# zacharie12/Hypernet-image-captioning

Hardware: AMD Instinct MI355X
Metric: training images/sec at 1/2/4/8 MI355X, Flickr30k GRU+hypernet bs=128 (higher is better)
Workload: dtype f32; 1 GPU; Flickr30k-shaped GRU+additive-attention decoder + hypernet (3 style domains), full training step (fwd, CE, bwd, clip 5.0, Adam); per_gpu_batch=128, global_batch=128, T=20, P=49, D=2048, F=200, E=200, H=200, V=9684, hypernet_params=144906720, parallelism=dp1, launch=eager, next_theta_in_adam_pass=True, next_precompute_beside_adam=True, spinup_steps=0, deterministic_gradients=True

## Files before the change

hypernet-image-captioning_amd/csrc/misc.hip:

```cpp
#include "common.h"
#include "gemm_internal.h"
#include <math.h>

namespace {
constexpr int RMAX = 8;


__global__ __launch_bounds__(256) void ce_count_kernel(int rows, const int64_t* __restrict__ tgt, int64_t ignore, float* nvalid) {
    __shared__ int cnt[4];
    int c = 0;
    for (int i = threadIdx.x; i < rows; i += 256) c += (tgt[i] != ignore);
    float cf = wave_sum((float)c);
    if ((threadIdx.x & 63) == 0) cnt[threadIdx.x >> 6] = (int)cf;
    __syncthreads();
    if (threadIdx.x == 0) nvalid[0] = (float)(cnt[0] + cnt[1] + cnt[2] + cnt[3]);
}

__global__ __launch_bounds__(256) void ce_row_kernel(int V, int ld, const float* logits, const int64_t* __restrict__ tgt,
                                                     int64_t ignore, const float* __restrict__ nvalid, const int* __restrict__ nvi,
                                                     float* dlogits, float* __restrict__ row_loss, int vec) {
    __shared__ float red[4];
    __shared__ float bc[2];
    const int row = blockIdx.x, tid = threadIdx.x;
    const float* x = logits + (size_t)row * ld;
// ... 300 lines not shown
        } else {
            for (size_t i = base + tid; i < n && i < base + SUMSQ_CHUNK; i += 256) s += x[i] * x[i];
        }
        mine = (double)s;
    } else {
        int q = bid - nb_s;
        const int chunk = q % NORM_CHUNKS; q /= NORM_CHUNKS;
        const int pair = q % (R * R); q /= (R * R);
        const int which = q & 1, job = q >> 1;
        const GramJob& J = jobs.j[job];
        const int r = pair / R, sidx = pair % R;
        const float* u = which ? J.afac + (size_t)r * J.lda : J.gfac + (size_t)r * J.ldg;
        const float* v = which ? J.afac + (size_t)sidx * J.lda : J.gfac + (size_t)sidx * J.ldg;
        const int len = which ? J.k : J.rows;
        const int per = (len + NORM_CHUNKS - 1) / NORM_CHUNKS;
        const int i0 = chunk * per, i1 = min(len, i0 + per);
        int i = i0 + tid;
        for (; i + 7 * 256 < i1; i += 8 * 256) {
            float uu[8], vv[8];
#pragma unroll
            for (int e = 0; e < 8; ++e) { uu[e] = u[i + 256 * e]; vv[e] = v[i + 256 * e]; }
#pragma unroll
            for (int e = 0; e < 8; ++e) mine += (double)uu[e] * (double)vv[e];
        }
        for (; i < i1; i += 256) mine += (double)u[i] * (double)v[i];
    }
    mine = wave_sum_d(mine);
    if ((tid & 63) == 0) red[tid >> 6] = mine;
    __syncthreads();
    if (tid == 0) part[bid] = red[0] + red[1] + red[2] + red[3];
}
__device__ __forceinline__ float norm_finish(int nb_s, int R, int njobs, const double* __restrict__ part, double max_norm, double scale,
                                             double* red , float* norm_out) {
    const int tid = threadIdx.x;
    const double* gram = part + nb_s;
    double tot = 0.0;
    for (int i = tid; i < nb_s; i += 256) tot += part[i];
    const int npair = njobs * R * R;
    for (int i = tid; i < npair; i += 256) {
        const int job = i / (R * R), pair = i % (R * R);
        const double* gg = gram + (((size_t)job * 2 + 0) * R * R + pair) * NORM_CHUNKS;
        const double* aa = gram + (((size_t)job * 2 + 1) * R * R + pair) * NORM_CHUNKS;
        double sg = 0.0, sa = 0.0;
        for (int c = 0; c < NORM_CHUNKS; ++c) { sg += gg[c]; sa += aa[c]; }
        tot += sg * sa;
    }
    tot = wave_sum_d(tot);
    if ((tid & 63) == 0) red[tid >> 6] = tot;
    __syncthreads();
    const double t = red[0] + red[1] + red[2] + red[3];
    const double norm = scale * sqrt(t);
    double c = max_norm / (norm + 1e-6);
    if (c > 1.0) c = 1.0;
    *norm_out = (float)norm;
    return (float)(scale * c);
}
__global__ __launch_bounds__(256) void grad_norm_finish_kernel(int nb_s, int R, int njobs, const double* __restrict__ part,
                                                               double max_norm, double scale, float* __restrict__ coef_out) {
    __shared__ double red[5];
    float norm;
    const float c = norm_finish(nb_s, R, njobs, part, max_norm, scale, red, &norm);
    if (threadIdx.x == 0) { coef_out[0] = c; coef_out[1] = norm; }
}

struct AdamK { float lr_bc1, b1, b2, eps, sqrt_bc2; const float* dev; int zg = 0; };
__device__ __forceinline__ void adam_moments(float g, float& m, float& v, const AdamK& k) {
    m = m + (g - m) * (1.0f - k.b1);
    v = v * k.b2 + (1.0f - k.b2) * g * g;
}
__device__ __forceinline__ float adam_elem(float p, float g, float& m, float& v, const AdamK& k) {
    adam_moments(g, m, v, k);
    const float denom = sqrtf(v) / k.sqrt_bc2 + k.eps;
    return p - k.lr_bc1 * (m / denom);
}
__device__ __forceinline__ void adam_moments_rank1(float a, float r, float& m, float& v, const AdamK& k) {
#pragma clang fp contract(off)
    const float g = a * r;
    const float d = __builtin_fmaf(a, r, -m);
    m = __builtin_fmaf(1.0f - k.b1, d, m);
    const float t = (1.0f - k.b2) * g;
    const float vb = v * k.b2, tg = t * g;
    v = vb + tg;
}
__device__ __forceinline__ float adam_elem_rank1(float p, float a, float r, float& m, float& v, const AdamK& k) {
#pragma clang fp contract(off)
    adam_moments_rank1(a, r, m, v, k);
    const float denom = sqrtf(v) / k.sqrt_bc2 + k.eps;
    return __builtin_fmaf(-k.lr_bc1, m / denom, p);
}
__global__ __launch_bounds__(256) void adam_dense_kernel(size_t n, float* __restrict__ p, float* __restrict__ m, float* __restrict__ v,
                                                         const float* __restrict__ g, const float* __restrict__ coef, AdamK k, int vec) {
    const float c = coef[0];
    if (k.dev) { k.lr_bc1 = k.dev[0]; k.sqrt_bc2 = k.dev[1]; }
    const size_t stride = (size_t)gridDim.x * 256;
    if (vec) {
        f32x4* p4 = reinterpret_cast<f32x4*>(p); f32x4* m4 = reinterpret_cast<f32x4*>(m); f32x4* v4 = reinterpret_cast<f32x4*>(v);
        const f32x4* g4 = reinterpret_cast<const f32x4*>(g);
        const size_t n4 = n >> 2;
        for (size_t i = (size_t)blockIdx.x * 256 + threadIdx.x; i < n4; i += stride) {
            f32x4 pp = p4[i], mm = m4[i], vv = v4[i], gg = g4[i];
#pragma unroll
            for (int e = 0; e < 4; ++e) { float me = mm[e], ve = vv[e]; pp[e] = adam_elem(pp[e], gg[e] * c, me, ve, k); mm[e] = me; vv[e] = ve; }
            p4[i] = pp; m4[i] = mm; v4[i] = vv;
        }
        for (size_t i = (n4 << 2) + (size_t)blockIdx.x * 256 + threadIdx.x; i < n; i += stride) {
            float me = m[i], ve = v[i]; p[i] = adam_elem(p[i], g[i] * c, me, ve, k); m[i] = me; v[i] = ve;
        }
    } else {
        for (size_t i = (size_t)blockIdx.x * 256 + threadIdx.x; i < n; i += stride) {
            float me = m[i], ve = v[i]; p[i] = adam_elem(p[i], g[i] * c, me, ve, k); m[i] = me; v[i] = ve;
        }
    }
}

struct NormFin { const double* part; int nb_s, R, njobs; double max_norm, scale; float* coef_out;
                 int ce_rows; const float* ce_rowloss; const float* ce_nvalid; const int* ce_nvi; float* loss_out; };
__global__ __launch_bounds__(256) void adam_dense_clip_kernel(size_t n, float* __restrict__ p, float* __restrict__ m, float* __restrict__ v,
                                                              const float* __restrict__ g, NormFin nf, AdamK k, int vec) {
    __shared__ double red[5];
    float norm;
    const float c = norm_finish(nf.nb_s, nf.R, nf.njobs, nf.part, nf.max_norm, nf.scale, red, &norm);
    if (blockIdx.x == 0) {
        if (threadIdx.x == 0) { nf.coef_out[0] = c; nf.coef_out[1] = norm; }
        if (nf.ce_rows > 0) {
            __syncthreads();
            double s = 0.0;
            for (int i = threadIdx.x; i < nf.ce_rows; i += 256) s += (double)nf.ce_rowloss[i];
            s = wave_sum_d(s);
            if ((threadIdx.x & 63) == 0) red[threadIdx.x >> 6] = s;
            __syncthreads();
            if (threadIdx.x == 0) {
                const float nn = nf.ce_nvi ? (float)nf.ce_nvi[0] : nf.ce_nvalid[0];
                nf.loss_out[0] = (float)((red[0] + red[1] + red[2] + red[3]) / (double)nn); nf.loss_out[1] = nn;
            }
        }
    }
    if (k.dev) { k.lr_bc1 = k.dev[0]; k.sqrt_bc2 = k.dev[1]; }
    const size_t stride = (size_t)gridDim.x * 256;
    if (vec) {
        f32x4* p4 = reinterpret_cast<f32x4*>(p); f32x4* m4 = reinterpret_cast<f32x4*>(m); f32x4* v4 = reinterpret_cast<f32x4*>(v);
        const f32x4* g4 = reinterpret_cast<const f32x4*>(g);
        const size_t n4 = n >> 2;
        for (size_t i = (size_t)blockIdx.x * 256 + threadIdx.x; i < n4; i += stride) {
            f32x4 pp = p4[i], mm = m4[i], vv = v4[i], gg = g4[i];
#pragma unroll
            for (int e = 0; e < 4; ++e) { float me = mm[e], ve = vv[e]; pp[e] = adam_elem(pp[e], gg[e] * c, me, ve, k); mm[e] = me; vv[e] = ve; }
            p4[i] = pp; m4[i] = mm; v4[i] = vv;
        }
        for (size_t i = (n4 << 2) + (size_t)blockIdx.x * 256 + threadIdx.x; i < n; i += stride) {
            float me = m[i], ve = v[i]; p[i] = adam_elem(p[i], g[i] * c, me, ve, k); m[i] = me; v[i] = ve;
        }
    } else {
        for (size_t i = (size_t)blockIdx.x * 256 + threadIdx.x; i < n; i += stride) {
            float me = m[i], ve = v[i]; p[i] = adam_elem(p[i], g[i] * c, me, ve, k); m[i] = me; v[i] = ve;
        }
    }
}

struct NextGemv {
    const float* a; const float* bias; float* theta;
    float* pack = nullptr; int pH = 0, pHA = 0, ppitch = 0, phrows = 0;
};
__device__ __forceinline__ void next_store(const NextGemv& nx, int row, float v) {
    nx.theta[row] = v;
    if (nx.pack) {
        const int R = row / nx.pH, c = row - R * nx.pH, q = R / nx.pH, j = R - q * nx.pH;
        const int hh = j >= nx.pHA ? 1 : 0, kk = j - (hh ? nx.pHA : 0), nk = hh ? nx.pH - nx.pHA : nx.pHA;
        nx.pack[((size_t)hh * nx.phrows + (size_t)(q + 1) * nk + kk) * nx.ppitch + c] = v;
    }
}
struct RankLag {
    int L, store_mv;
    const float* row_ring; size_t row_stride;
    const float* col_ring; size_t col_stride;
    float* save_row; float* save_col;
};
template <int QMAX, int RB, bool NTL, bool NTS, bool MULTI, int LAG = 0>
__device__ __forceinline__ void adam_rank_rows(int R, int rows, int k, float* W, float* m, float* v,
                                               const float* gfac, size_t ldg, const float* afac, size_t lda,
                                               float c, const AdamK& K, int wave_g, int nwaves, int lane, NextGemv nx,
                                               const f32x4* a_s ,
                                               const RankLag* lg = nullptr, const f32x4* c_s = nullptr ) {
    static_assert(LAG == 0 || !MULTI, "the lagged pass is rank 1");
    const int k4 = k >> 2;
    f32x4 an[QMAX];
#pragma unroll
    for (int q = 0; q < QMAX; ++q) {
        const int cidx = lane + 64 * q;
        an[q] = (nx.a && cidx < k4) ? reinterpret_cast<const f32x4*>(nx.a)[cidx] : f32x4{0.f, 0.f, 0.f, 0.f};
    }
    f32x4 a1[QMAX];
#pragma unroll
    for (int q = 0; q < QMAX; ++q) {
        const int cidx = lane + 64 * q;
        a1[q] = (!MULTI && LAG != 2 && cidx < k4) ? reinterpret_cast<const f32x4*>(afac)[cidx] : f32x4{0.f, 0.f, 0.f, 0.f};
    }
    for (int row0 = wave_g * RB; row0 < rows; row0 += nwaves * RB) {
        f32x4 pp[RB][QMAX], mm[RB][QMAX], vv[RB][QMAX];
#pragma unroll
        for (int i = 0; i < RB; ++i) {
            const size_t base = (size_t)(row0 + i) * k;
#pragma unroll
            for (int q = 0; q < QMAX; ++q) {
                const int cidx = lane + 64 * q;
                if (row0 + i < rows && cidx < k4) {
                    const f32x4* pw = reinterpret_cast<const f32x4*>(W + base) + cidx;
                    const f32x4* pm = reinterpret_cast<const f32x4*>(m + base) + cidx;
                    const f32x4* pv = reinterpret_cast<const f32x4*>(v + base) + cidx;
                    if constexpr (LAG != 2) pp[i][q] = NTL ? __builtin_nontemporal_load(pw) : *pw;
                    mm[i][q] = NTL ? __builtin_nontemporal_load(pm) : *pm;
                    vv[i][q] = NTL ? __builtin_nontemporal_load(pv) : *pv;
                }
            }
        }
        float grs[RB][MULTI ? RMAX : 1];
#pragma unroll
        for (int i = 0; i < RB; ++i)
#pragma unroll
            for (int r = 0; r < (MULTI ? RMAX : 1); ++r)
                grs[i][r] = (LAG != 2 && r < R && row0 + i < rows) ? gfac[(size_t)r * ldg + row0 + i] : 0.f;
        float rrv[RB];
        if constexpr (LAG != 0) {
#pragma unroll
            for (int i = 0; i < RB; ++i)
                rrv[i] = (lane < lg->L && row0 + i < rows) ? lg->row_ring[(size_t)lane * lg->row_stride + row0 + i] : 0.f;
        }
        if constexpr (LAG == 1) {
            if (lg->save_row && lane == 0) {
#pragma unroll
                for (int i = 0; i < RB; ++i)
                    if (row0 + i < rows) lg->save_row[row0 + i] = grs[i][0] * c;
            }
        }
        if constexpr (!MULTI && LAG != 2) {
            if (K.zg && lane == 0) {
#pragma unroll
                for (int i = 0; i < RB; ++i)
                    if (row0 + i < rows) const_cast<float*>(gfac)[row0 + i] = 0.f;
            }
        }
        float dots[RB];
#pragma unroll
        for (int i = 0; i < RB; ++i) dots[i] = 0.f;
#pragma unroll
        for (int i = 0; i < RB; ++i) {
            if (row0 + i >= rows) continue;
            const size_t base = (size_t)(row0 + i) * k;
            if constexpr (LAG != 0) {
#pragma unroll 1
                for (int l = 0; l < lg->L; ++l) {
                    const float r = __int_as_float(__builtin_amdgcn_readlane(__float_as_int(rrv[i]), l));
#pragma unroll
                    for (int q = 0; q < QMAX; ++q) {
                        const int cidx = lane + 64 * q;
                        if (cidx < k4) {
                            const f32x4 al = c_s[l * k4 + cidx];
#pragma unroll
                            for (int e = 0; e < 4; ++e) { float me = mm[i][q][e], ve = vv[i][q][e]; adam_moments_rank1(al[e], r, me, ve, K); mm[i][q][e] = me; vv[i][q][e] = ve; }
                        }
                    }
                }
            }
            float dot = 0.f;
            float gr[MULTI ? RMAX : 1];
#pragma unroll
            for (int r = 0; r < (MULTI ? RMAX : 1); ++r) gr[r] = grs[i][r] * c;
#pragma unroll
            for (int q = 0; q < QMAX; ++q) {
                const int cidx = lane + 64 * q;
                if (cidx < k4) {
                    f32x4 g;
                    if constexpr (!MULTI) g = a1[q] * gr[0];
                    else {
                        g = f32x4{0.f, 0.f, 0.f, 0.f};
#pragma unroll
                        for (int r = 0; r < RMAX; ++r)
                            if (r < R)
                                g += (a_s ? a_s[r * k4 + cidx] : reinterpret_cast<const f32x4*>(afac + (size_t)r * lda)[cidx]) * gr[r];
                    }
                    f32x4 po = pp[i][q], mo = mm[i][q], vo = vv[i][q];
                    if constexpr (LAG == 2) {
                        f32x4* qm = reinterpret_cast<f32x4*>(m + base) + cidx;
                        f32x4* qv = reinterpret_cast<f32x4*>(v + base) + cidx;
                        if (NTS) { __builtin_nontemporal_store(mo, qm); __builtin_nontemporal_store(vo, qv); }
                        else { *qm = mo; *qv = vo; }
                    } else {
#pragma unroll
                        for (int e = 0; e < 4; ++e) {
                            float me = mo[e], ve = vo[e];
                            if constexpr (LAG != 0) po[e] = adam_elem_rank1(po[e], a1[q][e], gr[0], me, ve, K);
                            else po[e] = adam_elem(po[e], g[e], me, ve, K);
                            mo[e] = me; vo[e] = ve;
                        }
                        dot += po[0] * an[q][0] + po[1] * an[q][1] + po[2] * an[q][2] + po[3] * an[q][3];
                        f32x4* qw = reinterpret_cast<f32x4*>(W + base) + cidx;
                        f32x4* qm = reinterpret_cast<f32x4*>(m + base) + cidx;
                        f32x4* qv = reinterpret_cast<f32x4*>(v + base) + cidx;
                        if constexpr (LAG == 1) {
                            if (NTS) __builtin_nontemporal_store(po, qw); else *qw = po;
                            if (lg->store_mv) {
                                if (NTS) { __builtin_nontemporal_store(mo, qm); __builtin_nontemporal_store(vo, qv); }
                                else { *qm = mo; *qv = vo; }
                            }
                        } else {
                            if (NTS) { __builtin_nontemporal_store(po, qw); __builtin_nontemporal_store(mo, qm); __builtin_nontemporal_store(vo, qv); }
                            else { *qw = po; *qm = mo; *qv = vo; }
                        }
                    }
                }
            }
            if (nx.a) dots[i] = wave_sum(dot);
        }
        if (nx.a && lane == 0) {
            bool vec_ok = row0 + RB <= rows && ((reinterpret_cast<uintptr_t>(nx.theta + row0) & (sizeof(float) * RB - 1)) == 0) &&
                          (RB == 2 || RB == 4);
            if (vec_ok && nx.pack) vec_ok = (nx.pH % RB) == 0 && (nx.ppitch % RB) == 0 && (reinterpret_cast<uintptr_t>(nx.pack) & 15) == 0;
            if (vec_ok) {
                float vals[RB];
#pragma unroll
                for (int i = 0; i < RB; ++i) vals[i] = dots[i] + nx.bias[row0 + i];
                float* pd = nullptr;
                if (nx.pack) {
                    const int R = row0 / nx.pH, c = row0 - R * nx.pH, q = R / nx.pH, j = R - q * nx.pH;
                    const int hh = j >= nx.pHA ? 1 : 0, kk = j - (hh ? nx.pHA : 0), nk = hh ? nx.pH - nx.pHA : nx.pHA;
                    pd = nx.pack + ((size_t)hh * nx.phrows + (size_t)(q + 1) * nk + kk) * nx.ppitch + c;
                }
                if constexpr (RB == 4) {
                    const f32x4 v4 = {vals[0], vals[1], vals[2], vals[3]};
                    *reinterpret_cast<f32x4*>(nx.theta + row0) = v4;
                    if (pd) *reinterpret_cast<f32x4*>(pd) = v4;
                } else if constexpr (RB == 2) {
                    typedef float f32x2v __attribute__((ext_vector_type(2)));
                    const f32x2v v2 = {vals[0], vals[1]};
                    *reinterpret_cast<f32x2v*>(nx.theta + row0) = v2;
                    if (pd) *reinterpret_cast<f32x2v*>(pd) = v2;
                }
            } else {
#pragma unroll
                for (int i = 0; i < RB; ++i)
                    if (row0 + i < rows) next_store(nx, row0 + i, dots[i] + nx.bias[row0 + i]);
            }
        }
    }
}
template <int RB, bool NTL, bool NTS, int QMAX, bool MULTI>
__global__ __launch_bounds__(256) void adam_rank_kernel(int R, int rows, int k, float* W, float* m, float* v,
                                                        const float* gfac, size_t ldg, const float* afac, size_t lda,
                                                        const float* coef, AdamK K, int vec, NextGemv nx, int use_lds) {
    extern __shared__ __attribute__((aligned(16))) f32x4 a_lds[];
    const float c = coef[0];
    if (K.dev) { K.lr_bc1 = K.dev[0]; K.sqrt_bc2 = K.dev[1]; }
    if (vec && k <= 256 * QMAX) {
        const f32x4* a_s = nullptr;
        if (R > 1 && use_lds) {
            const int k4 = k >> 2;
            for (int i = threadIdx.x; i < R * k4; i += 256) {
                const int r = i / k4, cc = i - r * k4;
                a_lds[i] = reinterpret_cast<const f32x4*>(afac + (size_t)r * lda)[cc];
            }
            __syncthreads();
            a_s = a_lds;
        }
        const int wave_g = blockIdx.x * 4 + (threadIdx.x >> 6), nwaves = gridDim.x * 4, lane = threadIdx.x & 63;
        adam_rank_rows<QMAX, RB, NTL, NTS, MULTI>(R, rows, k, W, m, v, gfac, ldg, afac, lda, c, K, wave_g, nwaves, lane, nx, a_s);
    } else {
        const size_t n = (size_t)rows * k, stride = (size_t)gridDim.x * 256;
        for (size_t i = (size_t)blockIdx.x * 256 + threadIdx.x; i < n; i += stride) {
            const size_t row = i / k, col = i % k;
            float g = 0.f;
            for (int r = 0; r < R; ++r) g += gfac[(size_t)r * ldg + row] * afac[(size_t)r * lda + col];
            float me = m[i], ve = v[i]; W[i] = adam_elem(W[i], g * c, me, ve, K); m[i] = me; v[i] = ve;
        }
    }
}
template <int RB, int QMAX, int LAG>
__global__ __launch_bounds__(256) void adam_rank_lag_kernel(int rows, int k, float* W, float* m, float* v, const float* gfac,
                                                            const float* afac, const float* coef, AdamK K, NextGemv nx, RankLag lg) {
    extern __shared__ __attribute__((aligned(16))) f32x4 c_lds[];
    const float c = LAG == 2 ? 0.f : coef[0];
    if (K.dev) { K.lr_bc1 = K.dev[0]; K.sqrt_bc2 = K.dev[1]; }
    const int k4 = k >> 2;
    if (lg.L > 0) {
        for (int i = threadIdx.x; i < lg.L * k4; i += 256) {
            const int l = i / k4, cc = i - l * k4;
            c_lds[i] = reinterpret_cast<const f32x4*>(lg.col_ring + (size_t)l * lg.col_stride)[cc];
        }
        __syncthreads();
    }
    if (LAG == 1 && lg.save_col && blockIdx.x == 0)
        for (int i = threadIdx.x; i < k4; i += 256) reinterpret_cast<f32x4*>(lg.save_col)[i] = reinterpret_cast<const f32x4*>(afac)[i];
    const int wave_g = blockIdx.x * 4 + (threadIdx.x >> 6), nwaves = gridDim.x * 4, lane = threadIdx.x & 63;
    adam_rank_rows<QMAX, RB, true, true, false, LAG>(1, rows, k, W, m, v, gfac, 0, afac, 0, c, K, wave_g, nwaves, lane, nx, nullptr, &lg, c_lds);
}
struct RankJob { float* W; float* m; float* v; const float* gfac; size_t ldg; const float* afac; size_t lda; NextGemv nx; int rows, k; };
struct RankJobs { RankJob j[4]; };
template <int RB, bool NTL, bool NTS, int QMAX, bool MULTI>
__global__ __launch_bounds__(256) void adam_rank_jobs_kernel(int R, RankJobs jobs, const float* coef, AdamK K, int use_lds) {
    extern __shared__ __attribute__((aligned(16))) f32x4 a_lds[];
    const RankJob& J = jobs.j[blockIdx.y];
    if ((long)blockIdx.x * 4 * RB >= J.rows) return;
    const float c = coef[0];
    if (K.dev) { K.lr_bc1 = K.dev[0]; K.sqrt_bc2 = K.dev[1]; }
    const f32x4* a_s = nullptr;
    if (R > 1 && use_lds) {
        const int k4 = J.k >> 2;
        for (int i = threadIdx.x; i < R * k4; i += 256) {
            const int r = i / k4, cc = i - r * k4;
            a_lds[i] = reinterpret_cast<const f32x4*>(J.afac + (size_t)r * J.lda)[cc];
        }
        __syncthreads();
        a_s = a_lds;
    }
    const int wave_g = blockIdx.x * 4 + (threadIdx.x >> 6), nwaves = gridDim.x * 4, lane = threadIdx.x & 63;
    adam_rank_rows<QMAX, RB, NTL, NTS, MULTI>(R, J.rows, J.k, J.W, J.m, J.v, J.gfac, J.ldg, J.afac, J.lda, c, K, wave_g, nwaves, lane, J.nx, a_s);
}
template <bool NT, bool NTS>
__global__ __launch_bounds__(256) void adam_rank_long_kernel(int R, int rows, int k, float* __restrict__ W, float* __restrict__ m,
                                                             float* __restrict__ v, const float* __restrict__ gfac, size_t ldg,
                                                             const float* __restrict__ afac, size_t lda,
                                                             const float* __restrict__ coef, AdamK K, NextGemv nx) {
    const float c = coef[0];
    if (K.dev) { K.lr_bc1 = K.dev[0]; K.sqrt_bc2 = K.dev[1]; }
    constexpr int U = 8;
    const int lane = threadIdx.x & 63, wave_g = blockIdx.x * 4 + (threadIdx.x >> 6), nwaves = gridDim.x * 4;
    const float* __restrict__ na = nx.a;
    for (int r = wave_g; r < rows; r += nwaves) {
        const size_t base = (size_t)r * k;
        float gr[RMAX];
#pragma unroll
        for (int q = 0; q < RMAX; ++q) gr[q] = q < R ? gfac[(size_t)q * ldg + r] : 0.f;
        float dot = 0.f;
        int col = lane;
        for (; col + 64 * (U - 1) < k; col += 64 * U) {
            float w[U], mm[U], vv[U], a[U];
#pragma unroll
            for (int u = 0; u < U; ++u) {
                const size_t i = base + col + 64 * u;
                if (NT) { w[u] = __builtin_nontemporal_load(W + i); mm[u] = __builtin_nontemporal_load(m + i); vv[u] = __builtin_nontemporal_load(v + i); }
                else { w[u] = W[i]; mm[u] = m[i]; vv[u] = v[i]; }
                a[u] = afac[col + 64 * u];
            }
#pragma unroll
            for (int u = 0; u < U; ++u) {
                float g = gr[0] * a[u];
                for (int q = 1; q < R; ++q) g += gr[q] * afac[(size_t)q * lda + col + 64 * u];
                w[u] = adam_elem(w[u], g * c, mm[u], vv[u], K);
                if (na) dot += w[u] * na[col + 64 * u];
                const size_t i = base + col + 64 * u;
                if (NTS) { __builtin_nontemporal_store(w[u], W + i); __builtin_nontemporal_store(mm[u], m + i); __builtin_nontemporal_store(vv[u], v + i); }
                else { W[i] = w[u]; m[i] = mm[u]; v[i] = vv[u]; }
            }
        }
        for (; col < k; col += 64) {
            const size_t i = base + col;
            float g = 0.f;
            for (int q = 0; q < R; ++q) g += gr[q] * afac[(size_t)q * lda + col];
            float me = m[i], ve = v[i];
            const float wn = adam_elem(W[i], g * c, me, ve, K);
            W[i] = wn; m[i] = me; v[i] = ve;
            if (na) dot += wn * na[col];
        }
        if (na) {
            dot = wave_sum(dot);
            if (lane == 0) next_store(nx, r, dot + nx.bias[r]);
        }
    }
}
__global__ __launch_bounds__(256) void rowdot_kernel(int rows, int k, const float* __restrict__ W, NextGemv nx) {
    const int grp = threadIdx.x >> 3, s = threadIdx.x & 7;
    for (int r = blockIdx.x * 32 + grp; r < rows; r += gridDim.x * 32) {
        float sum = 0.f;
        for (int c = s; c < k; c += 8) sum += W[(size_t)r * k + c] * nx.a[c];
        sum += __shfl_xor(sum, 4, 64); sum += __shfl_xor(sum, 2, 64); sum += __shfl_xor(sum, 1, 64);
        if (s == 0) next_store(nx, r, sum + nx.bias[r]);
    }
// ... 382 lines not shown
extern "C" int caphn_adam_rank_f32(int R, int rows, int k, float* W, float* m, float* v,
                                   const float* gfac, size_t ldg, const float* afac, size_t lda,
                                   const float* coef, const caphn_adam_hparams* hp, caphn_stream_t stream) {
    return adam_rank_launch(R, rows, k, W, m, v, gfac, ldg, afac, lda, coef, hp, NextGemv{nullptr, nullptr, nullptr}, stream);
}
extern "C" int caphn_adam_rank_gemv_f32(int R, int rows, int k, float* W, float* m, float* v,
                                        const float* gfac, size_t ldg, const float* afac, size_t lda,
                                        const float* coef, const caphn_adam_hparams* hp,
                                        const float* next_a, const float* next_bias, float* next_theta,
                                        caphn_stream_t stream) {
    if (!next_a || !next_bias || !next_theta) return CAPHN_EINVAL;
    return adam_rank_launch(R, rows, k, W, m, v, gfac, ldg, afac, lda, coef, hp, NextGemv{next_a, next_bias, next_theta}, stream);
}

extern "C" int caphn_adam_rank_multi_f32(int R, int njobs, const caphn_rank_job* jobs, const float* coef, const caphn_adam_hparams* hp,
                                         caphn_stream_t stream) {
    if (njobs <= 0 || !jobs || !coef || !hp || hp->step < 1 || R <= 0 || R > RMAX || (hp->zero_gfac && R != 1)) return CAPHN_EINVAL;
    auto qclass = [](int k) { return k <= 256 ? 1 : k <= 512 ? 2 : k <= 1024 ? 4 : 8; };
    bool one = njobs >= 2 && njobs <= 4 && g_tune_adam != 0;
    int maxrows = 0; size_t a_bytes = 0;
    for (int i = 0; i < njobs; ++i) {
        const caphn_rank_job& j = jobs[i];
        if (j.rows <= 0 || j.k <= 0 || !j.W || !j.m || !j.v || !j.gfac || !j.afac) return CAPHN_EINVAL;
        if ((j.next_a != nullptr) != (j.next_theta != nullptr) || (j.next_a != nullptr) != (j.next_bias != nullptr)) return CAPHN_EINVAL;
        if (j.next_pack && (!j.next_a || j.pack_H <= 0 || j.pack_HA <= 0 || j.pack_HA > j.pack_H || j.pack_pitch < j.pack_H || j.pack_hrows <= 0 ||
                            (long)j.rows % ((long)j.pack_H * j.pack_H) != 0)) return CAPHN_EINVAL;
        const bool vec = (j.k % 4 == 0) && (j.lda % 4 == 0) && caphn_aligned16(j.W) && caphn_aligned16(j.m) && caphn_aligned16(j.v) &&
                         caphn_aligned16(j.afac) && (!j.next_a || caphn_aligned16(j.next_a));
        one = one && vec && j.k <= 2048 && qclass(j.k) == qclass(jobs[0].k) && ((j.next_a != nullptr) == (jobs[0].next_a != nullptr)) &&
              j.rows <= 4 * g_tune_adam_cap;
        maxrows = std::max(maxrows, j.rows);
        a_bytes = std::max(a_bytes, sizeof(float) * (size_t)R * j.k);
    }
    if (!one) {
        for (int i = 0; i < njobs; ++i) {
            const caphn_rank_job& j = jobs[i];
            int rc = adam_rank_launch(R, j.rows, j.k, j.W, j.m, j.v, j.gfac, j.ldg, j.afac, j.lda, coef, hp,
                                      NextGemv{j.next_a, j.next_bias, j.next_theta, j.next_pack, j.pack_H, j.pack_HA, j.pack_pitch, j.pack_hrows}, stream);
            if (rc != CAPHN_OK) return rc;
        }
        return CAPHN_OK;
    }
    RankJobs J;
    for (int i = 0; i < njobs; ++i) {
        const caphn_rank_job& j = jobs[i];
        J.j[i] = RankJob{j.W, j.m, j.v, j.gfac, j.ldg, j.afac, j.lda,
                         NextGemv{j.next_a, j.next_bias, j.next_theta, j.next_pack, j.pack_H, j.pack_HA, j.pack_pitch, j.pack_hrows}, j.rows, j.k};
    }
    const int use_lds = R > 1 && a_bytes <= 60 * 1024;
    const size_t shm = use_lds ? a_bytes : 0;
    const AdamK K = make_adam(hp);
    hipStream_t s = static_cast<hipStream_t>(stream);
    const int q = qclass(jobs[0].k);
    const bool gemv = jobs[0].next_a != nullptr;
    const int RB = gemv ? (q == 1 ? 4 : 2) : (g_tune_adam == 3 ? 1 : 2);
    const dim3 grid((unsigned)((maxrows + 4 * RB - 1) / (4 * RB)), (unsigned)njobs);
#define RANK_JOBS_Q(RBv, Q) do { \
        if (R == 1) hipLaunchKernelGGL((adam_rank_jobs_kernel<RBv, true, true, Q, false>), grid, dim3(256), shm, s, R, J, coef, K, use_lds); \
        else hipLaunchKernelGGL((adam_rank_jobs_kernel<RBv, true, true, Q, true>), grid, dim3(256), shm, s, R, J, coef, K, use_lds); } while (0)
#define RANK_JOBS(RBv) do { if (q == 1) RANK_JOBS_Q(RBv, 1); else if (q == 2) RANK_JOBS_Q(RBv, 2); else if (q == 4) RANK_JOBS_Q(RBv, 4); \
                            else RANK_JOBS_Q(RBv, 8); } while (0)
    if (RB == 4) RANK_JOBS(4); else if (RB == 2) RANK_JOBS(2); else RANK_JOBS(1);
#undef RANK_JOBS
#undef RANK_JOBS_Q
    return caphn_launch_status();
}

int g_tune_lazy_moments = 4;
extern "C" int caphn_lazy_moments_period(void) { return g_tune_lazy_moments; }
static int rank_lag_check(int R, int rows, int k, const float* W, const float* m, const float* v, const float* afac, const float* next_a,
                          const caphn_rank_lag* lag, bool settle) {
    if (R != 1 || rows <= 0 || k <= 0 || !m || !v || !lag || (!settle && (!W || !afac))) return CAPHN_EINVAL;
    if (lag->pending < 0 || lag->pending > CAPHN_LAG_MAX) return CAPHN_EINVAL;
    if (lag->pending > 0 && (!lag->row_ring || !lag->col_ring || lag->row_stride < (size_t)rows || lag->col_stride < (size_t)k)) return CAPHN_EINVAL;
    if (!settle && !lag->store_mv && (!lag->save_row || !lag->save_col || lag->pending >= CAPHN_LAG_MAX)) return CAPHN_EINVAL;
    if (k % 4 != 0 || !caphn_aligned16(m) || !caphn_aligned16(v) || (!settle && (!caphn_aligned16(W) || !caphn_aligned16(afac))) ||
        (next_a && !caphn_aligned16(next_a)) || (lag->pending > 0 && (!caphn_aligned16(lag->col_ring) || lag->col_stride % 4 != 0)) ||
        (!settle && lag->save_col && !caphn_aligned16(lag->save_col))) return CAPHN_EINVAL;
    if (k > 2048) return CAPHN_ELIMIT;
    return CAPHN_OK;
}
static int rank_lag_launch(int mode, int rows, int k, float* W, float* m, float* v, const float* gfac, const float* afac,
                           const float* coef, const AdamK& K, NextGemv nx, const caphn_rank_lag* lag, caphn_stream_t stream) {
    long nb = ((long)rows + 3) / 4;
    if (nb > g_tune_adam_cap) nb = g_tune_adam_cap;
    if (nb < 1) nb = 1;
    hipStream_t s = static_cast<hipStream_t>(stream);
    RankLag lg{lag->pending, mode == 2 ? 1 : lag->store_mv, lag->row_ring, lag->row_stride, lag->col_ring, lag->col_stride,
               mode == 2 ? nullptr : lag->save_row, mode == 2 ? nullptr : lag->save_col};
    const size_t shm = sizeof(float) * (size_t)lag->pending * k;
#define RANK_LAG_Q(RB, Q) do { \
        if (mode == 2) hipLaunchKernelGGL((adam_rank_lag_kernel<2, Q, 2>), dim3((unsigned)nb), dim3(256), shm, s, rows, k, W, m, v, gfac, afac, coef, K, nx, lg); \
        else hipLaunchKernelGGL((adam_rank_lag_kernel<RB, Q, 1>), dim3((unsigned)nb), dim3(256), shm, s, rows, k, W, m, v, gfac, afac, coef, K, nx, lg); } while (0)
    if (k <= 256) { if (nx.a) RANK_LAG_Q(4, 1); else RANK_LAG_Q(2, 1); }
    else if (k <= 512) RANK_LAG_Q(2, 2);
    else if (k <= 1024) RANK_LAG_Q(2, 4);
    else RANK_LAG_Q(2, 8);
#undef RANK_LAG_Q
    return caphn_launch_status();
}
extern "C" int caphn_adam_rank_lag_f32(int R, int rows, int k, float* W, float* m, float* v, const float* gfac, const float* afac,
                                       const float* coef, const caphn_adam_hparams* hp, const caphn_rank_lag* lag,
                                       const float* next_a, const float* next_bias, float* next_theta, caphn_stream_t stream) {
    if (!gfac || !coef || !hp || hp->step < 1) return CAPHN_EINVAL;
    if ((next_a != nullptr) != (next_theta != nullptr) || (next_a != nullptr) != (next_bias != nullptr)) return CAPHN_EINVAL;
    const int rc = rank_lag_check(R, rows, k, W, m, v, afac, next_a, lag, false);
    if (rc != CAPHN_OK) return rc;
    return rank_lag_launch(1, rows, k, W, m, v, gfac, afac, coef, make_adam(hp), NextGemv{next_a, next_bias, next_theta}, lag, stream);
}
extern "C" int caphn_adam_rank_lag_multi_f32(int R, int njobs, const caphn_rank_job* jobs, const caphn_rank_lag* lags, const float* coef,
                                             const caphn_adam_hparams* hp, caphn_stream_t stream) {
    if (njobs <= 0 || !jobs || !lags || !coef || !hp || hp->step < 1) return CAPHN_EINVAL;
    for (int i = 0; i < njobs; ++i) {
        const caphn_rank_job& j = jobs[i];
        if (!j.gfac) return CAPHN_EINVAL;
        if ((j.next_a != nullptr) != (j.next_theta != nullptr) || (j.next_a != nullptr) != (j.next_bias != nullptr)) return CAPHN_EINVAL;
        if (j.next_pack && (!j.next_a || j.pack_H <= 0 || j.pack_HA <= 0 || j.pack_HA > j.pack_H || j.pack_pitch < j.pack_H || j.pack_hrows <= 0 ||
                            (long)j.rows % ((long)j.pack_H * j.pack_H) != 0)) return CAPHN_EINVAL;
        const int rc = rank_lag_check(R, j.rows, j.k, j.W, j.m, j.v, j.afac, j.next_a, &lags[i], false);
        if (rc != CAPHN_OK) return rc;
    }
    const AdamK K = make_adam(hp);
    for (int i = 0; i < njobs; ++i) {
        const caphn_rank_job& j = jobs[i];
        const int rc = rank_lag_launch(1, j.rows, j.k, j.W, j.m, j.v, j.gfac, j.afac, coef, K,
                                       NextGemv{j.next_a, j.next_bias, j.next_theta, j.next_pack, j.pack_H, j.pack_HA, j.pack_pitch, j.pack_hrows},
                                       &lags[i], stream);
        if (rc != CAPHN_OK) return rc;
    }
    return CAPHN_OK;
}
extern "C" int caphn_adam_rank_settle_f32(int rows, int k, float* m, float* v, float beta1, float beta2, const caphn_rank_lag* lag,
                                          caphn_stream_t stream) {
    const int rc = rank_lag_check(1, rows, k, nullptr, m, v, nullptr, nullptr, lag, true);
    if (rc != CAPHN_OK) return rc;
    if (lag->pending == 0) return CAPHN_OK;
    AdamK K{};
    K.b1 = beta1; K.b2 = beta2;
    return rank_lag_launch(2, rows, k, nullptr, m, v, nullptr, nullptr, nullptr, K, NextGemv{nullptr, nullptr, nullptr}, lag, stream);
}

extern "C" int caphn_abi_version(void) { return 1; }
extern "C" int caphn_device_arch(char* buf, int buflen) {
    if (!buf || buflen <= 0) return CAPHN_EINVAL;
    int dev = 0;
    hipDeviceProp_t prop;
    if (hipGetDevice(&dev) != hipSuccess || hipGetDeviceProperties(&prop, dev) != hipSuccess) return CAPHN_ELAUNCH;
    int i = 0;
    for (; i < buflen - 1 && prop.gcnArchName[i] && prop.gcnArchName[i] != ':'; ++i) buf[i] = prop.gcnArchName[i];
    buf[i] = 0;
    return CAPHN_OK;
}

static size_t mt_norm_blocks(int nt, const size_t* n) {
    size_t b = 0;
    for (int i = 0; i < nt; ++i) b += (n[i] + SUMSQ_CHUNK - 1) / SUMSQ_CHUNK;
    return b;
}
extern "C" size_t caphn_grad_norm_multi_workspace_bytes(int ntensors, const size_t* n, int R, int njobs) {
    if (ntensors < 0 || (ntensors > 0 && !n) || R <= 0 || R > RMAX || njobs < 0 || njobs > CAPHN_MAX_HEADS) return 0;
    return sizeof(double) * (mt_norm_blocks(ntensors, n) + (size_t)njobs * 2 * R * R * NORM_CHUNKS);
}
extern "C" int caphn_grad_norm_multi(int ntensors, const float* const* g, const size_t* n, int R, int njobs, const int* rows,
                                     const int* k, const float* const* gfac, const size_t* ldg, const float* const* afac,
                                     const size_t* lda, double max_norm, double scale, float* coef_out, void* ws,
                                     caphn_stream_t stream) {
    if (ntensors < 0 || (ntensors > 0 && (!g || !n)) || R <= 0 || R > RMAX || njobs < 0 || njobs > CAPHN_MAX_HEADS || !coef_out || !ws ||
        ntensors + njobs == 0) return CAPHN_EINVAL;
    GramJobs jobs; jobs.n = njobs;
    for (int i = 0; i < njobs; ++i) {
        if (!rows || !k || !gfac || !ldg || !afac || !lda || rows[i] <= 0 || k[i] <= 0 || !gfac[i] || !afac[i]) return CAPHN_EINVAL;
        jobs.j[i] = GramJob{gfac[i], ldg[i], afac[i], lda[i], rows[i], k[i]};
    }
    for (int i = 0; i < ntensors; ++i) if (!g[i] || n[i] == 0) return CAPHN_EINVAL;
    hipStream_t s = static_cast<hipStream_t>(stream);
    const size_t nb_total = mt_norm_blocks(ntensors, n);
    const unsigned ngram = (unsigned)(njobs * 2 * R * R * NORM_CHUNKS);
    double* part = static_cast<double*>(ws);
    size_t done = 0;
    int t0 = 0;
// ... 78 lines not shown
```

Baseline: 89680 images/s.

## Split lagged rank-1 Adam into dedicated kernel with LDS-staged factors and pipelined ring

Moves the lagged rank-1 Adam update out of the generic adam_rank_rows template into a dedicated row routine. The new routine stages the column ring, current factor and next-theta vector in LDS, clamps indices to avoid divergent branches, and software-pipelines the ring replay with double-buffered fetches. It also vectorizes the moment updates and next-theta stores, adds occupancy launch bounds, and sizes the grid by rows per block. The intent is to cut global loads and latency in the hypernet Adam pass, at the cost of more LDS per block, possibly above 64KB, and added register pressure.

```diff
diff --git a/hypernet-image-captioning_amd/csrc/misc.hip b/hypernet-image-captioning_amd/csrc/misc.hip
--- a/hypernet-image-captioning_amd/csrc/misc.hip
+++ b/hypernet-image-captioning_amd/csrc/misc.hip
@@ -406,9 +406,19 @@
     const float vb = v * k.b2, tg = t * g;
     v = vb + tg;
 }
-__device__ __forceinline__ float adam_elem_rank1(float p, float a, float r, float& m, float& v, const AdamK& k) {
+__device__ __forceinline__ void adam_moments_rank1_x4(const f32x4& a, float r, f32x4& m, f32x4& v, const AdamK& k) {
 #pragma clang fp contract(off)
-    adam_moments_rank1(a, r, m, v, k);
+    const float omb1 = 1.0f - k.b1, omb2 = 1.0f - k.b2;
+    const f32x4 r4 = {r, r, r, r}, c1 = {omb1, omb1, omb1, omb1}, c2 = {omb2, omb2, omb2, omb2}, b2 = {k.b2, k.b2, k.b2, k.b2};
+    const f32x4 g = a * r4;
+    const f32x4 d = __builtin_elementwise_fma(a, r4, -m);
+    m = __builtin_elementwise_fma(c1, d, m);
+    const f32x4 t = c2 * g;
+    const f32x4 vb = v * b2, tg = t * g;
+    v = vb + tg;
+}
+__device__ __forceinline__ float adam_apply_rank1(float p, float m, float v, const AdamK& k) {
+#pragma clang fp contract(off)
     const float denom = sqrtf(v) / k.sqrt_bc2 + k.eps;
     return __builtin_fmaf(-k.lr_bc1, m / denom, p);
 }
@@ -493,19 +503,48 @@
         nx.pack[((size_t)hh * nx.phrows + (size_t)(q + 1) * nk + kk) * nx.ppitch + c] = v;
     }
 }
+template <int RB>
+__device__ __forceinline__ void next_store_rows(const NextGemv& nx, int row0, int rows, const float* dots) {
+    bool vec_ok = row0 + RB <= rows && ((reinterpret_cast<uintptr_t>(nx.theta + row0) & (sizeof(float) * RB - 1)) == 0) &&
+                  (RB == 2 || RB == 4);
+    if (vec_ok && nx.pack) vec_ok = (nx.pH % RB) == 0 && (nx.ppitch % RB) == 0 && (reinterpret_cast<uintptr_t>(nx.pack) & 15) == 0;
+    if (vec_ok) {
+        float vals[RB];
+#pragma unroll
+        for (int i = 0; i < RB; ++i) vals[i] = dots[i] + nx.bias[row0 + i];
+        float* pd = nullptr;
+        if (nx.pack) {
+            const int R = row0 / nx.pH, c = row0 - R * nx.pH, q = R / nx.pH, j = R - q * nx.pH;
+            const int hh = j >= nx.pHA ? 1 : 0, kk = j - (hh ? nx.pHA : 0), nk = hh ? nx.pH - nx.pHA : nx.pHA;
+            pd = nx.pack + ((size_t)hh * nx.phrows + (size_t)(q + 1) * nk + kk) * nx.ppitch + c;
+        }
+        if constexpr (RB == 4) {
+            const f32x4 v4 = {vals[0], vals[1], vals[2], vals[3]};
+            *reinterpret_cast<f32x4*>(nx.theta + row0) = v4;
+            if (pd) *reinterpret_cast<f32x4*>(pd) = v4;
+        } else if constexpr (RB == 2) {
+            typedef float f32x2v __attribute__((ext_vector_type(2)));
+            const f32x2v v2 = {vals[0], vals[1]};
+            *reinterpret_cast<f32x2v*>(nx.theta + row0) = v2;
+            if (pd) *reinterpret_cast<f32x2v*>(pd) = v2;
+        }
+    } else {
+#pragma unroll
+        for (int i = 0; i < RB; ++i)
+            if (row0 + i < rows) next_store(nx, row0 + i, dots[i] + nx.bias[row0 + i]);
+    }
+}
 struct RankLag {
     int L, store_mv;
     const float* row_ring; size_t row_stride;
     const float* col_ring; size_t col_stride;
     float* save_row; float* save_col;
 };
-template <int QMAX, int RB, bool NTL, bool NTS, bool MULTI, int LAG = 0>
+template <int QMAX, int RB, bool NTL, bool NTS, bool MULTI>
 __device__ __forceinline__ void adam_rank_rows(int R, int rows, int k, float* W, float* m, float* v,
                                                const float* gfac, size_t ldg, const float* afac, size_t lda,
                                                float c, const AdamK& K, int wave_g, int nwaves, int lane, NextGemv nx,
-                                               const f32x4* a_s ,
-                                               const RankLag* lg = nullptr, const f32x4* c_s = nullptr ) {
-    static_assert(LAG == 0 || !MULTI, "the lagged pass is rank 1");
+                                               const f32x4* a_s ) {
     const int k4 = k >> 2;
     f32x4 an[QMAX];
 #pragma unroll
@@ -517,7 +556,7 @@
 #pragma unroll
     for (int q = 0; q < QMAX; ++q) {
         const int cidx = lane + 64 * q;
-        a1[q] = (!MULTI && LAG != 2 && cidx < k4) ? reinterpret_cast<const f32x4*>(afac)[cidx] : f32x4{0.f, 0.f, 0.f, 0.f};
+        a1[q] = (!MULTI && cidx < k4) ? reinterpret_cast<const f32x4*>(afac)[cidx] : f32x4{0.f, 0.f, 0.f, 0.f};
     }
     for (int row0 = wave_g * RB; row0 < rows; row0 += nwaves * RB) {
         f32x4 pp[RB][QMAX], mm[RB][QMAX], vv[RB][QMAX];
@@ -531,7 +570,7 @@
                     const f32x4* pw = reinterpret_cast<const f32x4*>(W + base) + cidx;
                     const f32x4* pm = reinterpret_cast<const f32x4*>(m + base) + cidx;
                     const f32x4* pv = reinterpret_cast<const f32x4*>(v + base) + cidx;
-                    if constexpr (LAG != 2) pp[i][q] = NTL ? __builtin_nontemporal_load(pw) : *pw;
+                    pp[i][q] = NTL ? __builtin_nontemporal_load(pw) : *pw;
                     mm[i][q] = NTL ? __builtin_nontemporal_load(pm) : *pm;
                     vv[i][q] = NTL ? __builtin_nontemporal_load(pv) : *pv;
                 }
@@ -542,21 +581,8 @@
         for (int i = 0; i < RB; ++i)
 #pragma unroll
             for (int r = 0; r < (MULTI ? RMAX : 1); ++r)
-                grs[i][r] = (LAG != 2 && r < R && row0 + i < rows) ? gfac[(size_t)r * ldg + row0 + i] : 0.f;
-        float rrv[RB];
-        if constexpr (LAG != 0) {
-#pragma unroll
-            for (int i = 0; i < RB; ++i)
-                rrv[i] = (lane < lg->L && row0 + i < rows) ? lg->row_ring[(size_t)lane * lg->row_stride + row0 + i] : 0.f;
-        }
-        if constexpr (LAG == 1) {
-            if (lg->save_row && lane == 0) {
-#pragma unroll
-                for (int i = 0; i < RB; ++i)
-                    if (row0 + i < rows) lg->save_row[row0 + i] = grs[i][0] * c;
-            }
-        }
-        if constexpr (!MULTI && LAG != 2) {
+                grs[i][r] = (r < R && row0 + i < rows) ? gfac[(size_t)r * ldg + row0 + i] : 0.f;
+        if constexpr (!MULTI) {
             if (K.zg && lane == 0) {
 #pragma unroll
                 for (int i = 0; i < RB; ++i)
@@ -570,21 +596,6 @@
         for (int i = 0; i < RB; ++i) {
             if (row0 + i >= rows) continue;
             const size_t base = (size_t)(row0 + i) * k;
-            if constexpr (LAG != 0) {
-#pragma unroll 1
-                for (int l = 0; l < lg->L; ++l) {
-                    const float r = __int_as_float(__builtin_amdgcn_readlane(__float_as_int(rrv[i]), l));
-#pragma unroll
-                    for (int q = 0; q < QMAX; ++q) {
-                        const int cidx = lane + 64 * q;
-                        if (cidx < k4) {
-                            const f32x4 al = c_s[l * k4 + cidx];
-#pragma unroll
-                            for (int e = 0; e < 4; ++e) { float me = mm[i][q][e], ve = vv[i][q][e]; adam_moments_rank1(al[e], r, me, ve, K); mm[i][q][e] = me; vv[i][q][e] = ve; }
-                        }
-                    }
-                }
-            }
             float dot = 0.f;
             float gr[MULTI ? RMAX : 1];
 #pragma unroll
@@ -603,34 +614,14 @@
                                 g += (a_s ? a_s[r * k4 + cidx] : reinterpret_cast<const f32x4*>(afac + (size_t)r * lda)[cidx]) * gr[r];
                     }
                     f32x4 po = pp[i][q], mo = mm[i][q], vo = vv[i][q];
-                    if constexpr (LAG == 2) {
-                        f32x4* qm = reinterpret_cast<f32x4*>(m + base) + cidx;
-                        f32x4* qv = reinterpret_cast<f32x4*>(v + base) + cidx;
-                        if (NTS) { __builtin_nontemporal_store(mo, qm); __builtin_nontemporal_store(vo, qv); }
-                        else { *qm = mo; *qv = vo; }
-                    } else {
-#pragma unroll
-                        for (int e = 0; e < 4; ++e) {
-                            float me = mo[e], ve = vo[e];
-                            if constexpr (LAG != 0) po[e] = adam_elem_rank1(po[e], a1[q][e], gr[0], me, ve, K);
-                            else po[e] = adam_elem(po[e], g[e], me, ve, K);
-                            mo[e] = me; vo[e] = ve;
-                        }
-                        dot += po[0] * an[q][0] + po[1] * an[q][1] + po[2] * an[q][2] + po[3] * an[q][3];
-                        f32x4* qw = reinterpret_cast<f32x4*>(W + base) + cidx;
-                        f32x4* qm = reinterpret_cast<f32x4*>(m + base) + cidx;
-                        f32x4* qv = reinterpret_cast<f32x4*>(v + base) + cidx;
-                        if constexpr (LAG == 1) {
-                            if (NTS) __builtin_nontemporal_store(po, qw); else *qw = po;
-                            if (lg->store_mv) {
-                                if (NTS) { __builtin_nontemporal_store(mo, qm); __builtin_nontemporal_store(vo, qv); }
-                                else { *qm = mo; *qv = vo; }
-                            }
-                        } else {
-                            if (NTS) { __builtin_nontemporal_store(po, qw); __builtin_nontemporal_store(mo, qm); __builtin_nontemporal_store(vo, qv); }
-                            else { *qw = po; *qm = mo; *qv = vo; }
-                        }
-                    }
+#pragma unroll
+                    for (int e = 0; e < 4; ++e) { float me = mo[e], ve = vo[e]; po[e] = adam_elem(po[e], g[e], me, ve, K); mo[e] = me; vo[e] = ve; }
+                    dot += po[0] * an[q][0] + po[1] * an[q][1] + po[2] * an[q][2] + po[3] * an[q][3];
+                    f32x4* qw = reinterpret_cast<f32x4*>(W + base) + cidx;
+                    f32x4* qm = reinterpret_cast<f32x4*>(m + base) + cidx;
+                    f32x4* qv = reinterpret_cast<f32x4*>(v + base) + cidx;
+                    if (NTS) { __builtin_nontemporal_store(po, qw); __builtin_nontemporal_store(mo, qm); __builtin_nontemporal_store(vo, qv); }
+                    else { *qw = po; *qm = mo; *qv = vo; }
                 }
             }
             if (nx.a) dots[i] = wave_sum(dot);
@@ -697,24 +688,149 @@
         }
     }
 }
+template <int QMAX, int RB, int LAG>
+__device__ __forceinline__ void adam_rank_lag_rows(int rows, int k, float* W, float* m, float* v, const float* gfac, float c,
+                                                   const AdamK& K, int wave_g, int nwaves, int lane, const NextGemv& nx,
+                                                   const RankLag& lg, const f32x4* c_s ,
+                                                   const f32x4* a_s , const f32x4* n_s ) {
+    const int k4 = k >> 2, L = lg.L;
+    int cq[QMAX];
+#pragma unroll
+    for (int q = 0; q < QMAX; ++q) cq[q] = min(lane + 64 * q, k4 - 1);
+    const float* rr = L > 0 ? lg.row_ring + (size_t)min(lane, L - 1) * lg.row_stride : gfac;
+    for (int row0 = wave_g * RB; row0 < rows; row0 += nwaves * RB) {
+        f32x4 pp[RB][QMAX], mm[RB][QMAX], vv[RB][QMAX];
+        int rc[RB];
+        float rrv[RB], grs[RB];
+#pragma unroll
+        for (int i = 0; i < RB; ++i) {
+            rc[i] = min(row0 + i, rows - 1);
+            rrv[i] = rr[rc[i]];
+            grs[i] = LAG != 2 ? gfac[rc[i]] : 0.f;
+        }
+#pragma unroll
+        for (int i = 0; i < RB; ++i)
+#pragma unroll
+            for (int q = 0; q < QMAX; ++q) {
+                mm[i][q] = __builtin_nontemporal_load(reinterpret_cast<const f32x4*>(m + (size_t)rc[i] * k) + cq[q]);
+                vv[i][q] = __builtin_nontemporal_load(reinterpret_cast<const f32x4*>(v + (size_t)rc[i] * k) + cq[q]);
+            }
+        if constexpr (LAG != 2) {
+            __builtin_amdgcn_sched_barrier(0);
+#pragma unroll
+            for (int i = 0; i < RB; ++i)
+#pragma unroll
+                for (int q = 0; q < QMAX; ++q)
+                    pp[i][q] = __builtin_nontemporal_load(reinterpret_cast<const f32x4*>(W + (size_t)rc[i] * k) + cq[q]);
+        }
+        {
+            f32x4 fa[QMAX], fb[QMAX];
+            float ra[RB], rb[RB];
+            auto fetch = [&](f32x4 (&f)[QMAX], float (&r)[RB], int l) {
+#pragma unroll
+                for (int q = 0; q < QMAX; ++q) f[q] = c_s[l * k4 + cq[q]];
+#pragma unroll
+                for (int i = 0; i < RB; ++i) r[i] = __int_as_float(__builtin_amdgcn_readlane(__float_as_int(rrv[i]), l));
+            };
+            auto apply = [&](const f32x4 (&f)[QMAX], const float (&r)[RB]) {
+#pragma unroll
+                for (int i = 0; i < RB; ++i)
+#pragma unroll
+                    for (int q = 0; q < QMAX; ++q) adam_moments_rank1_x4(f[q], r[i], mm[i][q], vv[i][q], K);
+            };
+            fetch(fa, ra, 0);
+#pragma unroll 1
+            for (int l = 0; l + 1 < L; l += 2) {
+                fetch(fb, rb, l + 1);
+                apply(fa, ra);
+                fetch(fa, ra, min(l + 2, L - 1));
+                apply(fb, rb);
+            }
+            if (L & 1) apply(fa, ra);
+        }
+        if constexpr (LAG == 2) {
+#pragma unroll
+            for (int i = 0; i < RB; ++i)
+#pragma unroll
+                for (int q = 0; q < QMAX; ++q)
+                    if (row0 + i < rows && lane + 64 * q < k4) {
+                        __builtin_nontemporal_store(mm[i][q], reinterpret_cast<f32x4*>(m + (size_t)(row0 + i) * k) + lane + 64 * q);
+                        __builtin_nontemporal_store(vv[i][q], reinterpret_cast<f32x4*>(v + (size_t)(row0 + i) * k) + lane + 64 * q);
+                    }
+        } else {
+            if (lane == 0) {
+#pragma unroll
+                for (int i = 0; i < RB; ++i)
+                    if (row0 + i < rows) {
+                        if (lg.save_row) lg.save_row[row0 + i] = grs[i] * c;
+                        if (K.zg) const_cast<float*>(gfac)[row0 + i] = 0.f;
+                    }
+            }
+            float dots[RB];
+#pragma unroll
+            for (int i = 0; i < RB; ++i) {
+                const float gr = grs[i] * c;
+                float dot = 0.f;
+#pragma unroll
+                for (int q = 0; q < QMAX; ++q) {
+                    const bool live = row0 + i < rows && lane + 64 * q < k4;
+                    f32x4 po = pp[i][q];
+                    adam_moments_rank1_x4(a_s[cq[q]], gr, mm[i][q], vv[i][q], K);
+                    const f32x4 mo = mm[i][q], vo = vv[i][q];
+#pragma unroll
+                    for (int e = 0; e < 4; ++e) po[e] = adam_apply_rank1(po[e], mo[e], vo[e], K);
+                    if (nx.a) {
+#pragma clang fp contract(off)
+                        const f32x4 an = n_s[cq[q]];
+                        const float t = po[0] * an[0] + po[1] * an[1] + po[2] * an[2] + po[3] * an[3];
+                        dot = live ? dot + t : dot;
+                    }
+                    if (live) {
+                        const size_t o = (size_t)(row0 + i) * k;
+                        __builtin_nontemporal_store(po, reinterpret_cast<f32x4*>(W + o) + lane + 64 * q);
+                        if (lg.store_mv) {
+                            __builtin_nontemporal_store(mo, reinterpret_cast<f32x4*>(m + o) + lane + 64 * q);
+                            __builtin_nontemporal_store(vo, reinterpret_cast<f32x4*>(v + o) + lane + 64 * q);
+                        }
+                    }
+                }
+                dots[i] = nx.a ? wave_sum(dot) : 0.f;
+            }
+            if (nx.a && lane == 0) next_store_rows<RB>(nx, row0, rows, dots);
+        }
+    }
+}
 template <int RB, int QMAX, int LAG>
-__global__ __launch_bounds__(256) void adam_rank_lag_kernel(int rows, int k, float* W, float* m, float* v, const float* gfac,
+__global__ __launch_bounds__(256, (RB * QMAX <= 4 ? 4 : 1)) void adam_rank_lag_kernel(int rows, int k, float* W, float* m, float* v, const float* gfac,
                                                             const float* afac, const float* coef, AdamK K, NextGemv nx, RankLag lg) {
     extern __shared__ __attribute__((aligned(16))) f32x4 c_lds[];
     const float c = LAG == 2 ? 0.f : coef[0];
     if (K.dev) { K.lr_bc1 = K.dev[0]; K.sqrt_bc2 = K.dev[1]; }
     const int k4 = k >> 2;
-    if (lg.L > 0) {
-        for (int i = threadIdx.x; i < lg.L * k4; i += 256) {
-            const int l = i / k4, cc = i - l * k4;
-            c_lds[i] = reinterpret_cast<const f32x4*>(lg.col_ring + (size_t)l * lg.col_stride)[cc];
-        }
-        __syncthreads();
-    }
-    if (LAG == 1 && lg.save_col && blockIdx.x == 0)
-        for (int i = threadIdx.x; i < k4; i += 256) reinterpret_cast<f32x4*>(lg.save_col)[i] = reinterpret_cast<const f32x4*>(afac)[i];
+    f32x4* a_s = c_lds + lg.L * k4;
+    f32x4* n_s = a_s + k4;
+    const float* ring = lg.L > 0 ? lg.col_ring : afac;
+    const size_t rs = lg.L > 0 ? lg.col_stride : 0;
+    for (int i = threadIdx.x; i < k4; i += 256) {
+        f32x4 t[CAPHN_LAG_MAX], a, n;
+#pragma unroll
+        for (int l = 0; l < CAPHN_LAG_MAX; ++l) t[l] = reinterpret_cast<const f32x4*>(ring + (size_t)min(l, max(lg.L - 1, 0)) * rs)[i];
+        if (LAG == 1) {
+            a = reinterpret_cast<const f32x4*>(afac)[i];
+            n = reinterpret_cast<const f32x4*>(nx.a ? nx.a : afac)[i];
+        }
+#pragma unroll
+        for (int l = 0; l < CAPHN_LAG_MAX; ++l)
+            if (l < lg.L) c_lds[l * k4 + i] = t[l];
+        if (LAG == 1) {
+            a_s[i] = a;
+            n_s[i] = n;
+            if (lg.save_col && blockIdx.x == 0) reinterpret_cast<f32x4*>(lg.save_col)[i] = a;
+        }
+    }
+    __syncthreads();
     const int wave_g = blockIdx.x * 4 + (threadIdx.x >> 6), nwaves = gridDim.x * 4, lane = threadIdx.x & 63;
-    adam_rank_rows<QMAX, RB, true, true, false, LAG>(1, rows, k, W, m, v, gfac, 0, afac, 0, c, K, wave_g, nwaves, lane, nx, nullptr, &lg, c_lds);
+    adam_rank_lag_rows<QMAX, RB, LAG>(rows, k, W, m, v, gfac, c, K, wave_g, nwaves, lane, nx, lg, c_lds, a_s, n_s);
 }
 struct RankJob { float* W; float* m; float* v; const float* gfac; size_t ldg; const float* afac; size_t lda; NextGemv nx; int rows, k; };
 struct RankJobs { RankJob j[4]; };
@@ -1263,20 +1379,23 @@
 }
 static int rank_lag_launch(int mode, int rows, int k, float* W, float* m, float* v, const float* gfac, const float* afac,
                            const float* coef, const AdamK& K, NextGemv nx, const caphn_rank_lag* lag, caphn_stream_t stream) {
-    long nb = ((long)rows + 3) / 4;
-    if (nb > g_tune_adam_cap) nb = g_tune_adam_cap;
-    if (nb < 1) nb = 1;
     hipStream_t s = static_cast<hipStream_t>(stream);
     RankLag lg{lag->pending, mode == 2 ? 1 : lag->store_mv, lag->row_ring, lag->row_stride, lag->col_ring, lag->col_stride,
                mode == 2 ? nullptr : lag->save_row, mode == 2 ? nullptr : lag->save_col};
-    const size_t shm = sizeof(float) * (size_t)lag->pending * k;
+    const size_t shm = sizeof(float) * (size_t)(lag->pending + (mode == 2 ? 0 : 2)) * k;
+#define RANK_LAG_K(KERN, RB) do { \
+        long nb = ((long)rows + 4 * RB - 1) / (4 * RB); \
+        if (nb > g_tune_adam_cap) nb = g_tune_adam_cap; \
+        if (shm > 64 * 1024 && hipFuncSetAttribute(reinterpret_cast<const void*>(&KERN), hipFuncAttributeMaxDynamicSharedMemorySize, (int)shm) != hipSuccess) \
+            return CAPHN_ELAUNCH; \
+        hipLaunchKernelGGL(KERN, dim3((unsigned)nb), dim3(256), shm, s, rows, k, W, m, v, gfac, afac, coef, K, nx, lg); } while (0)
 #define RANK_LAG_Q(RB, Q) do { \
-        if (mode == 2) hipLaunchKernelGGL((adam_rank_lag_kernel<2, Q, 2>), dim3((unsigned)nb), dim3(256), shm, s, rows, k, W, m, v, gfac, afac, coef, K, nx, lg); \
-        else hipLaunchKernelGGL((adam_rank_lag_kernel<RB, Q, 1>), dim3((unsigned)nb), dim3(256), shm, s, rows, k, W, m, v, gfac, afac, coef, K, nx, lg); } while (0)
+        if (mode == 2) RANK_LAG_K((adam_rank_lag_kernel<2, Q, 2>), 2); else RANK_LAG_K((adam_rank_lag_kernel<RB, Q, 1>), RB); } while (0)
     if (k <= 256) { if (nx.a) RANK_LAG_Q(4, 1); else RANK_LAG_Q(2, 1); }
     else if (k <= 512) RANK_LAG_Q(2, 2);
     else if (k <= 1024) RANK_LAG_Q(2, 4);
     else RANK_LAG_Q(2, 8);
+#undef RANK_LAG_K
 #undef RANK_LAG_Q
     return caphn_launch_status();
 }
```

New measurement: 90510 images/s, median of 6. No clear change (+0.9%).
